# ucsdarclab/Python-SuPer

Measured on AMD Instinct MI355X. Metric: LM iterations/s (embedded-deformation LM, point-to-plane + ARAP + Rot), higher is better.
Workload: dtype f64

## Files before the change

python-super_amd/csrc/slm_api.hip:

```cpp
#include <atomic>
#include <condition_variable>
#include <functional>
#include <mutex>
#include <new>
#include <string>
#include <thread>
#include <algorithm>
#include <vector>
#include <cstdio>
#include <cstring>

#include "slm_common.h"
#include "slm_corr.h"
#include "slm_host.h"
#include "slm_launch.h"
#include "slm_prep.h"

static thread_local std::string g_err;
static const char* const kBadKnn =
    "slm_bind_frame: a KNN index (sf_knn_idx or ed_knn_idx) lies outside [0, J) or a surfel's row of sf_knn_idx repeats an id";

void slm_set_error_text(const char* msg) { g_err = msg; }

namespace {
// ... 195 lines not shown
  void ensure(int n_workers) {
    while ((int)threads_.size() < n_workers) {
      const int id = (int)threads_.size();
      threads_.emplace_back([this, id] { loop(id); });
    }
  }
  void loop(int id) {
    int seen = 0;
    for (;;) {
      const std::function<void(int)>* job = nullptr;
      {
        std::unique_lock<std::mutex> lk(m_);
        cv_work_.wait(lk, [&] { return stop_ || generation_ != seen; });
        if (stop_) return;
        seen = generation_;
        if (id < n_active_) job = job_;
      }
      if (job) {
        (*job)(id + 1);
        std::lock_guard<std::mutex> lk(m_);
        if (--pending_ == 0) cv_done_.notify_all();
      }
    }
  }
  std::vector<std::thread> threads_;
  std::mutex m_;
  std::condition_variable cv_work_, cv_done_;
  const std::function<void(int)>* job_ = nullptr;
  int generation_ = 0, n_active_ = 0, pending_ = 0;
  bool stop_ = false;
};
}

struct slm_solver {
  PrepBuffers* prep = nullptr;
  BindPool bind_pool;
  AsyncWorker prep_worker;
  PrepBuffers* prep_async = nullptr;
  hipStream_t prep_stream = nullptr;
  std::vector<PrepBuffers*> bind_prep;
  std::vector<hipStream_t> bind_streams;
  std::vector<hipEvent_t> bind_events;
  std::mutex band_mutex;
  hipEvent_t drain_event = nullptr;
  double drain_est_ms = 0.0;
  int last_solver_form = -1;
  int last_dag_mode = -1;
  bool no_reuse = false;
  bool hybrid_batches = true;
  long dag_max_nodes = 8000;
  bool fuse_begin = true;
  int gram_wgs = 0;
  int n_cus = 256;
  bool pure_fill = true;
  bool profile = false;
  std::vector<hipEvent_t> ev_pool;
  std::vector<std::vector<hipEvent_t>> ev_runs;
  slm_config cfg{};
  std::vector<Slot> slots;
  FrameDev* frames_dev = nullptr;
  int* bw_dev = nullptr;
  int* bw_host = nullptr;
  int* reuse_dev = nullptr;
  int rank = 0, world = 1;
  int corr_mode = 0;
  double corr_w = 0.0;
  CorrDev* corr_dev = nullptr;
  bool shard_mode = false;
};
namespace {
bool solve_is_task_graph(const slm_solver* s, int n, int J);
}

static std::atomic<long long> g_reallocs{0}, g_realloc_bytes{0}, g_plan_builds{0}, g_plan_reuses{0}, g_plan_fill_hits{0};

template <typename T>
static hipError_t grow(T*& p, size_t& cap, size_t need) {
  if (need <= cap) return hipSuccess;
  const size_t want = need + need / 8;
  ++g_reallocs;
  g_realloc_bytes += (long long)(want * sizeof(T));
  return grow(p, cap, need, want);
}
template <typename T>
static hipError_t grow(GP<T>& p, size_t& cap, size_t need) {
  T* q = p;
  const hipError_t e = grow(q, cap, need);
  p = q;
  return e;
}

static int check_slots(slm_solver* s, int first, int n);

extern "C" {

const char* slm_last_error(void) { return g_err.c_str(); }

int slm_debug_last_solver_form(slm_solver* s) { return s ? s->last_solver_form : -1; }
int slm_debug_last_dag_mode(slm_solver* s) { return s ? s->last_dag_mode : -1; }

int slm_debug_counters(int64_t out[4]) {
  if (!out) return fail(SLM_ERR_INVALID, "slm_debug_counters: null output");
  out[0] = g_reallocs;
  out[1] = g_realloc_bytes;
  out[2] = g_plan_builds;
  out[3] = g_plan_reuses;
// ... 107 lines not shown
    return fail(SLM_ERR_INVALID, buf);
  }
  return SLM_OK;
}

int slm_device_count(void) {
  int n = 0;
  if (hipGetDeviceCount(&n) != hipSuccess) return 0;
  return n;
}

int slm_create(const slm_config* cfg, slm_solver** out) {
  if (!cfg || !out) return fail(SLM_ERR_INVALID, "slm_create: null argument");
  if (cfg->max_frames < 1 || cfg->num_iterations < 0 || !(cfg->v > 0.0))
    return fail(SLM_ERR_INVALID, "slm_create: bad config");
  if (cfg->solver_path < 0 || cfg->solver_path > 4) return fail(SLM_ERR_INVALID, "slm_create: solver_path must be 0..4");
  if (cfg->data_path < 0 || cfg->data_path > 2) return fail(SLM_ERR_INVALID, "slm_create: data_path must be 0..2");
  if (slm_device_count() < 1) return fail(SLM_ERR_NO_DEVICE, "slm_create: no HIP device visible");
  slm_solver* s = new (std::nothrow) slm_solver();
  if (!s) return fail(SLM_ERR_HIP, "slm_create: out of host memory");
  s->cfg = *cfg;
  try {
    s->slots.resize(cfg->max_frames);
  } catch (...) {
    delete s;
    return fail(SLM_ERR_HIP, "slm_create: out of host memory");
  }
  hipError_t e = hipMalloc((void**)&s->frames_dev, sizeof(FrameDev) * cfg->max_frames);
  if (e == hipSuccess) e = hipMemset(s->frames_dev, 0, sizeof(FrameDev) * cfg->max_frames);
  if (e == hipSuccess) e = hipMalloc((void**)&s->bw_dev, 2 * sizeof(int));
  if (e == hipSuccess) e = hipMalloc((void**)&s->reuse_dev, sizeof(int) * cfg->max_frames);
  if (e == hipSuccess) e = hipMemset(s->reuse_dev, 0, sizeof(int) * cfg->max_frames);
  if (e == hipSuccess) e = hipHostMalloc((void**)&s->bw_host, 2 * sizeof(int), hipHostMallocDefault);
  if (e == hipSuccess) {
    s->prep = prep_create();
    if (!s->prep) e = hipErrorOutOfMemory;
  }
  if (e != hipSuccess) {
    g_err = std::string("slm_create: ") + hipGetErrorString(e);
    slm_destroy(s);
    return SLM_ERR_HIP;
  }
  {
    int dev = 0;
    (void)hipGetDevice(&dev);
    (void)dag_device_setup(dev, nullptr);
  }
  if (const char* hb = getenv("SLM_HYBRID")) s->hybrid_batches = atoi(hb) != 0;
  if (const char* dm = getenv("SLM_DAG_MAX_NODES")) s->dag_max_nodes = atol(dm);
  if (const char* nr = getenv("SLM_NO_REUSE")) s->no_reuse = atoi(nr) != 0;
  if (const char* pf = getenv("SLM_PURE_FILL")) s->pure_fill = atoi(pf) != 0;
  if (const char* fb = getenv("SLM_FUSE_BEGIN")) s->fuse_begin = atoi(fb) != 0;
  if (const char* gw = getenv("SLM_GRAM_WGS")) s->gram_wgs = std::min(std::max(atoi(gw), 0), 65535);
  {
    int dev = 0, cus = 0;
    (void)hipGetDevice(&dev);
    if (hipDeviceGetAttribute(&cus, hipDeviceAttributeMultiprocessorCount, dev) == hipSuccess && cus > 0) s->n_cus = cus;
  }
  *out = s;
  return SLM_OK;
}

int slm_destroy(slm_solver* s) {
  if (!s) return SLM_OK;
  s->prep_worker.shutdown();
  s->bind_pool.shutdown();
  for (Slot& sl : s->slots) {
    FrameDev& h = sl.h;
    if (h.beta) (void)hipFree(h.beta);
    if (h.delta) (void)hipFree(h.delta);
    if (h.rhs) (void)hipFree(h.rhs);
    if (sl.band) (void)hipFree(sl.band);
    if (sl.linv) (void)hipFree(sl.linv);
    if (h.loss_part) (void)hipFree(h.loss_part);
    if (h.st) (void)hipFree(h.st);
    if (h.rec) (void)hipFree(h.rec);
    if (h.node_pk) (void)hipFree(h.node_pk);
    if (h.tgt_pn) (void)hipFree(h.tgt_pn);
    if (h.tgt_px) (void)hipFree(h.tgt_px);
    if (h.ev_rc) (void)hipFree(h.ev_rc);
    plan_free(sl.plan);
    pairplan_free(sl.pplan);
    if (sl.h_pin) (void)hipHostFree(sl.h_pin);
    sl.h_pairs.release();
    sl.h_knn.release();
    sl.h_pts.release();
    sl.h_pts64.release();
    if (sl.d_fronts) (void)hipFree(sl.d_fronts);
    if (sl.d_items) (void)hipFree(sl.d_items);
    if (sl.d_tile_kind) (void)hipFree(sl.d_tile_kind);
    if (sl.d_zero_tiles) (void)hipFree(sl.d_zero_tiles);
    if (sl.d_ints) (void)hipFree(sl.d_ints);
    if (sl.d_dests) (void)hipFree(sl.d_dests);
    if (sl.d_cur_dests) (void)hipFree(sl.d_cur_dests);
    if (sl.ftiles) (void)hipFree(sl.ftiles);
    if (sl.fvec) (void)hipFree(sl.fvec);
    if (sl.flinv) (void)hipFree(sl.flinv);
    if (sl.fmail) (void)hipFree(sl.fmail);
    if (sl.pairbuf) (void)hipFree(sl.pairbuf);
    if (sl.corr.o) (void)hipFree(sl.corr.o);
    if (sl.corr.n) (void)hipFree(sl.corr.n);
    if (sl.corr.valid) (void)hipFree(sl.corr.valid);
    if (sl.d_dag_flags) (void)hipFree(sl.d_dag_flags);
    if (sl.d_dag_trace) (void)hipFree(sl.d_dag_trace);
    if (sl.prep_fork) (void)hipEventDestroy(sl.prep_fork);
    if (sl.prep_done) (void)hipEventDestroy(sl.prep_done);
// ... 704 lines not shown
  d.fused_begin = d.nd && tuple && d.gram_variants == 1 && d.max_pos > 0 && s->fuse_begin;
  if (tuple && c.phase_test) d.accept_reuse = s->reuse_dev + first;
  d.accept_eval = tuple ? 1 : 0;
  if (d.nd) {
    for (int i = first; i < first + n; ++i) {
      const auto& sc = s->slots[i].cache.nd.sched;
      if (sc.size() > d.sched.size()) d.sched.resize(sc.size(), NDLevelSched{0, 0, 0, 0, 0, -2, 0, -2, 0, -2});
      for (size_t l = 0; l < sc.size(); ++l) {
        NDLevelSched& m = d.sched[l];
        if (m.first == -2) m.first = sc[l].first;
        else if (m.first != sc[l].first || m.n_fronts != sc[l].n_fronts) m.first = -1;
        m.n_fronts = std::max(m.n_fronts, sc[l].n_fronts);
        m.max_npt = std::max(m.max_npt, sc[l].max_npt);
        m.max_nt = std::max(m.max_nt, sc[l].max_nt);
        m.max_pairs = std::max(m.max_pairs, sc[l].max_pairs);
        m.max_n2p = std::max(m.max_n2p, sc[l].max_n2p);
        if (m.schur_at == -2) m.schur_at = sc[l].schur_at;
        else if (m.schur_at != sc[l].schur_at || m.n_schur != sc[l].n_schur) m.schur_at = -1;
        m.n_schur = std::max(m.n_schur, sc[l].n_schur);
        if (m.pull_at == -2) m.pull_at = sc[l].pull_at;
        else if (m.pull_at != sc[l].pull_at || m.n_pull != sc[l].n_pull) m.pull_at = -1;
        m.n_pull = std::max(m.n_pull, sc[l].n_pull);
      }
    }
  }
  if (d.nd && n > 1) {
    for (int i = first; i < first + n; ++i)
      for (size_t l = s->slots[i].cache.nd.sched.size(); l < d.sched.size(); ++l)
        d.sched[l].first = d.sched[l].schur_at = d.sched[l].pull_at = -1;
  }
  for (auto& m : d.sched) {
    if (m.first == -2) m.first = -1;
    if (m.first < 0) m.schur_at = m.pull_at = -1;
    if (m.schur_at == -2) m.schur_at = -1;
    if (m.pull_at == -2) m.pull_at = -1;
  }
  if (s->cfg.use_arap || s->cfg.use_rot)
    d.n_reg_part = std::min(kRegBlocksMax, (d.maxJKe + 255) / 256);
  d.n_acc_part = d.n_reg_part + (s->corr_mode ? kCorrBlocks : 0);
  return d;
}

static bool solve_is_task_graph(const slm_solver* s, int n, int J) {
  return s->cfg.solver_path == 2 || (s->cfg.solver_path == 0 && (n <= 2 || (long)n * J <= s->dag_max_nodes));
}
static bool solve_is_hybrid(const slm_solver* s, int n, const BatchDims& d) {
  return !solve_is_task_graph(s, n, d.maxP / 7) && (s->cfg.solver_path == 4 || (s->cfg.solver_path == 0 && s->hybrid_batches)) &&
         d.hybrid_cut >= 0 && d.hybrid_levels == (int)d.sched.size() && d.hybrid_cut + 1 < d.hybrid_levels;
}
static int dag_cut_of(const slm_solver* s, int n, const BatchDims& d) {
  if (solve_is_task_graph(s, n, d.maxP / 7)) return -1;
  return solve_is_hybrid(s, n, d) ? d.hybrid_cut : -2;
}
int enqueue_front_solve(slm_solver* s, const FrameDev* fr, int n, const BatchDims& d, double u_override, hipStream_t st,
                        bool dag_reset_done = false, bool dag_check_later = false) {
  const bool dag = solve_is_task_graph(s, n, d.maxP / 7);
  const bool hybrid = solve_is_hybrid(s, n, d);
  s->last_solver_form = dag ? 1 : (hybrid ? 2 : 0);
  int mode = -1;
  if (dag) {
    mode = launch_front_solve_dag(fr, n, d.max_tasks, u_override, st, -1, !dag_reset_done, !dag_check_later);
  } else if (hybrid) {
    const int n_levels = (int)d.sched.size(), l_cut = n_levels - 1 - d.hybrid_cut;
    launch_front_levels(fr, n, d.sched.data(), n_levels, l_cut, 0, u_override, st);
    mode = launch_front_solve_dag(fr, n, d.max_top_tasks, u_override, st, d.hybrid_cut, !dag_reset_done, !dag_check_later);
  } else {
    launch_front_solve(fr, n, d.sched.data(), (int)d.sched.size(), u_override, st);
  }
  s->last_dag_mode = mode;
  return mode;
}

void enqueue_zero(const FrameDev* fr, int n, const BatchDims& d, hipStream_t st, const int* reuse, int dag_cut, bool fused) {
  if (!d.nd) launch_iter_begin(fr, n, st);
  else if (!fused) launch_iter_begin_nd(fr, n, st, reuse, dag_cut);
}

void enqueue_jacobian(slm_solver* s, const FrameDev* fr, int n, const BatchDims& d, hipStream_t st, int eval_mode,
                      const int* reuse, int dag_cut, bool fused) {
  const double w = s->cfg.w_data;
  switch (d.form) {
    case DataForm::tuple:
      if (eval_mode >= 0) launch_data_eval(fr, n, kLossBlocks, w, eval_mode, st, reuse);
      if (fused) launch_begin_and_gram(fr, n, w, st, reuse, dag_cut, s->gram_wgs, s->n_cus);
      else launch_data_gram(fr, n, d.max_pos, w, d.gram_variants, st, reuse, s->gram_wgs, s->n_cus);
      break;
    case DataForm::pairs:
      launch_data_grad_pairs(fr, n, d.maxN, d.K, w, st);
      if (d.corr) launch_corr_grad_pairs(fr, s->corr_dev + (fr - s->frames_dev), n, d.maxN, d.K, s->corr_mode, s->corr_w, st);
      break;
    case DataForm::per_entry:
      launch_data_grad(fr, n, d.maxN, d.K, w, st);
      if (d.corr) launch_corr_grad(fr, s->corr_dev + (fr - s->frames_dev), n, d.maxN, d.K, s->corr_mode, s->corr_w, st);
      break;
    case DataForm::none: break;
  }
}

enum class Shard { whole, before_exchange, after_exchange };
void enqueue_scatter(slm_solver* s, const FrameDev* fr, int n, const BatchDims& d, hipStream_t st, Shard part) {
  const slm_config& c = s->cfg;
  const bool tuple = d.form == DataForm::tuple;
  if (part == Shard::before_exchange) {
    if (tuple) launch_pair_reduce(fr, n, d.max_blocks, st);
    return;
  }
  if (part == Shard::after_exchange || d.form == DataForm::pairs) launch_pair_scatter(fr, n, d.max_blocks, st);
  else if (tuple && d.nd) launch_front_assemble(fr, n, d.max_blocks, st);
  else if (tuple) launch_band_assemble(fr, n, d.max_blocks, st);
  if (d.nd) {
    launch_reg_grad_nd(fr, n, d.maxP / 7, c.use_arap, c.w_arap, c.use_rot, c.w_rot, st);
    if (!c.use_arap && !c.use_rot) launch_front_load_rhs(fr, n, d.maxP, st);
  } else {
    launch_reg_grad(fr, n, d.maxJKe, c.use_arap, c.w_arap, c.use_rot, c.w_rot, st);
  }
}

void enqueue_data_loss(slm_solver* s, const FrameDev* fr, int n, const BatchDims& d, hipStream_t st, bool at_beta) {
  if (d.form == DataForm::tuple && !at_beta) launch_data_eval(fr, n, kLossBlocks, s->cfg.w_data, 0, st);
  else if (d.form != DataForm::none) launch_data_loss(fr, n, kLossBlocks, d.K, s->cfg.w_data, at_beta ? 0 : 1, st);
// ... 630 lines not shown
```

python-super_amd/csrc/slm_front.hip:

```cpp
#include <algorithm>
#include <atomic>
#include <cstdlib>

#include "slm_tile.h"
#include "slm_begin.h"
#include "slm_launch.h"

__device__ __forceinline__ int nd_base(const NDFront& f, int p) {
  return p < f.nv ? 7 * p : f.n1p + 7 * (p - f.nv);
}

__device__ __forceinline__ double* ftile(const FrameDev& fd, const NDFront& f, int r, int c) {
  const size_t t = (size_t)c * f.nt - (size_t)c * (c - 1) / 2 + (size_t)(r - c);
  return fd.ftiles + f.tile_off + t * TILE;
}

__device__ __forceinline__ double* front_entry(const FrameDev& fd, const NDFront& f, int i, int j) {
  return ftile(fd, f, i >> 6, j >> 6) + (i & 63) + (size_t)(j & 63) * NB;
}

__device__ __forceinline__ double* dest_entry(const FrameDev& fd, const NDDest& d, int x, int y) {
  const NDFront& f = fd.fronts[d.front];
  const int rb = nd_base(f, d.prow), cb = nd_base(f, d.pcol);
  return d.transpose ? front_entry(fd, f, rb + y, cb + x) : front_entry(fd, f, rb + x, cb + y);
// ... 385 lines not shown
                                                 int c, double u_override, WgMap map) {
  extern __shared__ double lds[];
  double *S = PanelLds::S(lds), *M = PanelLds::M(lds), *dinv = PanelLds::dinv(lds), *vec = PanelLds::vec(lds);
  LevelCtx cx;
  if (!level_begin(frames, lvl, c, map, cx)) return;
  const FrameDev& fd = *cx.fd;
  const NDFront& f = *cx.f;
  const int d = cx.unit;
  if (c + d >= f.nt) return;
  const double u = (u_override >= 0.0) ? u_override : fd.st->u;
  const bool stamp = (c == 1 && cx.frame == 0 && cx.front == 0 && d == 1 && lvl.level == fd.n_levels - 1);
  SLM_STAMP(fd, stamp, 0);
  double* At = ftile(fd, f, c + d, c);
  double* yv = fd.fvec + f.vec_off + (size_t)c * NB;
  double4_t a[4];
  panel_column_stage(d, At, yv, ftile(fd, f, c, c), c * NB, f.n1, u, S, vec, a);
  SLM_STAMP(fd, stamp, 1);
  const bool ok = PanelLds::factor(lds, nullptr, nullptr, nullptr, min(4, (f.n1 - c * NB + 15) >> 4));
  SLM_STAMP(fd, stamp, 14);
  if (d == 0 && !ok && threadIdx.x == 0) fd.st->chol_fail = 1;
  panel_column_finish(d, At, yv, fd.flinv + f.linv_off + (size_t)c * TILE, S, M, dinv, vec, a);
  SLM_STAMP(fd, stamp, 15);
}

__global__ void __launch_bounds__(256) k_fpotrf(const FrameDev* __restrict__ frames, LevelRef lvl, int c,
                                                 double u_override) {
  extern __shared__ double lds[];
  double *S = PanelLds::S(lds), *M = PanelLds::M(lds), *dinv = PanelLds::dinv(lds), *vec = PanelLds::vec(lds);
  LevelCtx cx;
  if (!level_begin(frames, lvl, c, cx)) return;
  const FrameDev& fd = *cx.fd;
  const NDFront& f = *cx.f;
  const double u = (u_override >= 0.0) ? u_override : fd.st->u;
  double* yv = fd.fvec + f.vec_off + (size_t)c * NB;
  double4_t a[4];
  panel_column_stage(0, nullptr, yv, ftile(fd, f, c, c), c * NB, f.n1, u, S, vec, a);
  const bool ok = PanelLds::factor(lds, nullptr, nullptr, nullptr, min(4, (f.n1 - c * NB + 15) >> 4));
  if (!ok && threadIdx.x == 0) fd.st->chol_fail = 1;
  panel_column_finish(0, nullptr, yv, fd.flinv + f.linv_off + (size_t)c * TILE, S, M, dinv, vec, a);
}

__global__ void __launch_bounds__(256) k_ftrsm(const FrameDev* __restrict__ frames, LevelRef lvl, int c, WgMap map) {
  __shared__ double Bl[TILE];
  LevelCtx cx;
  if (!level_begin(frames, lvl, c, map, cx)) return;
  const FrameDev& fd = *cx.fd;
  const NDFront& f = *cx.f;
  const int d = cx.unit + 1;
  if (c + d >= f.nt) return;
  double* At = ftile(fd, f, c + d, c);
  tile_product<false, true, false>(fd.flinv + f.linv_off + (size_t)c * TILE, At, At, Bl);
}

__device__ __forceinline__ const NDTileItem* tile_item(const FrameDev* __restrict__ frames, int level, int which, int n_items,
                                                       int at, int n_frames, const FrameDev*& fdp) {
  const int total = n_items * n_frames;
  const int chunk = (total + 7) >> 3;
  const int q = blockIdx.x >> 3;
  const int w_id = (blockIdx.x & 7) * chunk + q;
  if (q >= chunk || w_id >= total) return nullptr;
  const int frame = w_id / n_items, item_idx = w_id - frame * n_items;
  const FrameDev& fd = frames[frame];
  if (!fd.bound || !fd.nd_ready) return nullptr;
  int i0 = at;
  if (at < 0) {
    if (level >= fd.n_levels) return nullptr;
    i0 = fd.item_off[2 * level + which];
    if (item_idx >= fd.item_off[2 * level + which + 1] - i0) return nullptr;
  }
  fdp = &fd;
  return fd.tile_items.get() + i0 + item_idx;
}
__device__ __forceinline__ NDTileItem item_snapshot(const NDTileItem* p) {
  NDTileItem o;
  const int* src = reinterpret_cast<const int*>(p);
  int* dst = reinterpret_cast<int*>(&o);
#pragma unroll
  for (int i = 0; i < (int)(sizeof(NDTileItem) / 4); ++i) dst[i] = __builtin_amdgcn_readfirstlane(src[i]);
  return o;
}
__device__ __forceinline__ double* item_tile(const FrameDev& fd, const NDTileItem& it, int r, int c) {
  const size_t t = (size_t)c * it.nt - (size_t)c * (c - 1) / 2 + (size_t)(r - c);
  return fd.ftiles + (c < it.npt ? it.tile_off : it.f22_base) + t * TILE;
}
__device__ __forceinline__ void pull_maps(const FrameDev& fd, const NDTileItem& it, int2* maps) {
#pragma unroll
  for (int k = 0; k < 2; ++k) {
    if (it.kid[k].front >= 0 && threadIdx.x < 128) {
      const int32_t* pm = fd.pullmap + it.kid[k].pull_off;
      const bool row = threadIdx.x < 64;
      const int c = pm[64 * (row ? it.r : it.c) + (threadIdx.x & 63)];
      int off = 0;
      if (c >= 0) {
        const int t = it.kid[k].npt + (c >> 6);
        off = row ? t * TILE + (c & 63) : (t * it.kid[k].nt - t * (t - 1) / 2 - t) * TILE + (c & 63) * NB;
      }
      maps[128 * k + threadIdx.x] = make_int2(c, off);
    }
  }
}
__device__ __forceinline__ void pull_tile(const FrameDev& fd, const NDTileItem& it, const int2* maps, double4_t acc[4]) {
  const int l = threadIdx.x & 63, w = threadIdx.x >> 6, lr = l & 15, lk = l >> 4;
#pragma unroll
  for (int k = 0; k < 2; ++k) {
    if (it.kid[k].front < 0) continue;
    __builtin_amdgcn_sched_barrier(0);
    double v[16];
    const double* ct = fd.ftiles + it.kid[k].f22_base;
    const int2* mk = maps + 128 * k;
    const int2 rw = mk[16 * w + lr];
#pragma unroll
    for (int ni = 0; ni < 4; ++ni)
#pragma unroll
      for (int rr = 0; rr < 4; ++rr) {
        const int2 cl = mk[64 + 16 * ni + lk + 4 * rr];
        const bool ok = cl.x >= 0 && rw.x >= cl.x;
        const double x = ct[ok ? rw.y + cl.y : 0];
        v[4 * ni + rr] = ok ? x : 0.0;
      }
    __builtin_amdgcn_sched_barrier(0);
#pragma unroll
    for (int ni = 0; ni < 4; ++ni)
#pragma unroll
      for (int rr = 0; rr < 4; ++rr) acc[ni][rr] += v[4 * ni + rr];
    __builtin_amdgcn_sched_barrier(0);
  }
}
__device__ __forceinline__ double pull_vec(const FrameDev& fd, const NDTileItem& it, const int2* maps) {
  double s = 0.0;
  if (threadIdx.x < NB) {
#pragma unroll
    for (int k = 0; k < 2; ++k) {
      if (it.kid[k].front < 0) continue;
      const int ci = maps[128 * k + threadIdx.x].x;
      if (ci >= 0) s += fd.fvec[it.kid[k].vec_boundary + ci];
    }
  }
  return s;
}

__global__ void __launch_bounds__(256, 2) k_fL11(const FrameDev* __restrict__ frames, LevelRef lvl,
                                               double u_override) {
  extern __shared__ double lds[];
  double *S = L11Lds::S(lds), *M = L11Lds::M(lds);
  double* Bl = L11Lds::Bl(lds);
  double* vec = L11Lds::vec(lds);
  double* part = L11Lds::vec2(lds);
  LevelCtx cx;
  if (!level_begin(frames, lvl, 0, cx)) return;
  const FrameDev& fd = *cx.fd;
  const NDFront& f = *cx.f;
  const double u = (u_override >= 0.0) ? u_override : fd.st->u;
  double* vecs = fd.fvec + f.vec_off;
  const int w = threadIdx.x >> 6, l = threadIdx.x & 63, lr = l & 15, lk = l >> 4;

  for (int c = 0; c < f.npt; ++c) {
    double rhs_c = 0.0;
    {
      double v[16];
      tile_to_regs(ftile(fd, f, c, c), v);
      if (threadIdx.x < NB) rhs_c = vecs[(size_t)c * NB + threadIdx.x];
#pragma unroll
      for (int t = 0; t < 16; ++t) {
        const int e = threadIdx.x + 256 * t;
        const int i = e % NB, k = e / NB;
        double x = (i >= k) ? v[t] : 0.0;
        if (i == k) x = (c * NB + i < f.n1) ? x + u : 1.0;
        S[i + k * LD] = x;
      }
    }
    __syncthreads();
    const bool ok = L11Lds::factor(lds, nullptr, nullptr, nullptr, min(4, (f.n1 - c * NB + 15) >> 4));
    if (!ok && threadIdx.x == 0) fd.st->chol_fail = 1;
    if (threadIdx.x < NB) vec[threadIdx.x] = rhs_c;
    __syncthreads();
    {
      commit_pivot(M, vec, fd.flinv + f.linv_off + (size_t)c * TILE, part);
      __syncthreads();
      if (threadIdx.x < NB) {
        vec[threadIdx.x] = part[threadIdx.x];
        vecs[(size_t)c * NB + threadIdx.x] = part[threadIdx.x];
      }
      __syncthreads();
    }
    for (int r = c + 1; r < f.npt; ++r) {
      double* At = ftile(fd, f, r, c);
      double areg[16];
// ... 91 lines not shown
  LevelCtx cx;
  if (!level_begin(frames, lvl, c, map, cx)) return;
  const FrameDev& fd = *cx.fd;
  const NDFront& f = *cx.f;
  const int m = f.nt - 1 - c;
  int t = cx.unit;
  if (t < ntile_cap) {
    int db = 1;
    while (db <= bcap && t >= mcap - db + 1) {
      t -= mcap - db + 1;
      ++db;
    }
    const int da = db + t;
    if (da > m || c + db >= f.npt) return;
    tile_product<true, false, true>(ftile(fd, f, c + db, c), ftile(fd, f, c + da, c), ftile(fd, f, c + da, c + db), Bl);
  } else {
    const int db = t - ntile_cap + 1;
    if (db > m) return;
    __shared__ double y[NB];
    __shared__ double part[4 * NB];
    double* vecs = fd.fvec + f.vec_off;
    trail_rhs(ftile(fd, f, c + db, c), vecs + (size_t)c * NB, vecs + (size_t)(c + db) * NB, y, part);
  }
}

__global__ void __launch_bounds__(256) k_fpull(const FrameDev* __restrict__ frames, int level, int n_items, int items_at,
                                                int n_frames) {
  __shared__ int2 maps[256];
  const FrameDev* fdp;
  const NDTileItem* itp = tile_item(frames, level, 1, n_items, items_at, n_frames, fdp);
  if (!itp) return;
  const FrameDev& fd = *fdp;
  const NDTileItem it = item_snapshot(itp);
  const int w = threadIdx.x >> 6;
  const int vrow = it.r < it.npt ? min(NB, it.n1 - NB * it.r) : min(NB, it.n2 - NB * (it.r - it.npt));
  const int nblk = (min(NB, it.n1 - NB * it.c) + 15) >> 4;
  const bool wave_on = 16 * w < vrow;
  pull_maps(fd, it, maps);
  double* T = item_tile(fd, it, it.r, it.c);
  const bool pure = __builtin_amdgcn_readfirstlane((int)fd.tile_kind[it.pad0]) != 0;
  double4_t acc[4];
  zero_acc(acc);
  if (wave_on && !pure) load_c_frags_nblk(T, acc, nblk);
  __syncthreads();
  if (wave_on) pull_tile(fd, it, maps, acc);
  if (pure) store_c_frags(T, acc);
  else if (wave_on) store_c_frags_nblk(T, acc, nblk);
  if (it.r == it.c) {
    const double v = pull_vec(fd, it, maps);
    if (threadIdx.x < NB && v != 0.0) fd.fvec[it.vec_off + (size_t)it.c * NB + threadIdx.x] += v;
  }
}

__global__ void __launch_bounds__(256, 3) k_fschur(const FrameDev* __restrict__ frames, int level, int n_items,
                                                 int items_at, int n_frames) {
  __shared__ __attribute__((aligned(16))) double Bl[TILE];
  __shared__ int2 maps[256];
  const FrameDev* fdp;
  const NDTileItem* itp = tile_item(frames, level, 0, n_items, items_at, n_frames, fdp);
  if (!itp) return;
  const FrameDev& fd = *fdp;
  const NDTileItem& it = *itp;
  const int r = it.r, sc = it.c, tr = r - it.npt, tc = sc - it.npt;
  const int l = threadIdx.x & 63, w = threadIdx.x >> 6, lr = l & 15, lk = l >> 4;
  const int vrow = min(NB, it.n2 - NB * tr), vcol = min(NB, it.n2 - NB * tc);
  const bool wave_on = 16 * w < vrow;
  const int nblk = (tr == tc) ? min((vcol + 15) >> 4, w + 1) : (vcol + 15) >> 4;
  const bool kids = it.kid[0].front >= 0 || it.kid[1].front >= 0;
  pull_maps(fd, it, maps);
  typedef double dvec2 __attribute__((ext_vector_type(2)));
  dvec2 breg[4];
  double areg[16], acur[16];
  if (it.npt > 0) {
    const dvec2* Ls = reinterpret_cast<const dvec2*>(item_tile(fd, it, sc, 0));
#pragma unroll
    for (int e = 0; e < 4; ++e) breg[e] = Ls[threadIdx.x + 256 * e];
    if (wave_on) load_a_frags(item_tile(fd, it, r, 0), areg);
  }
  double4_t acc[4];
  zero_acc(acc);
  __syncthreads();
  if (kids) pull_tile(fd, it, maps, acc);
  for (int c = 0; c < it.npt; ++c) {
    const dvec2* Ls = reinterpret_cast<const dvec2*>(item_tile(fd, it, sc, c));
    dvec2* Bl2 = reinterpret_cast<dvec2*>(Bl);
    const int ksteps = min(16, (it.n1 - NB * c + 3) >> 2);
#pragma unroll
    for (int e = 0; e < 4; ++e) Bl2[threadIdx.x + 256 * e] = breg[e];
#pragma unroll
    for (int e = 0; e < 16; ++e) acur[e] = areg[e];
    if (ksteps > 8) {
#pragma unroll
      for (int e = 0; e < 4; ++e) breg[e] = Ls[TILE / 4 + threadIdx.x + 256 * e];
    }
    if (c + 1 < it.npt && wave_on) load_a_frags(item_tile(fd, it, r, c + 1), areg);
    __syncthreads();
    if (wave_on) {
#pragma unroll
      for (int ks = 0; ks < 8; ++ks) {
        if (ks < ksteps) {
          const double av = -acur[ks];
#pragma unroll
          for (int ni = 0; ni < 4; ++ni)
            if (ni < nblk)
              acc[ni] = __builtin_amdgcn_mfma_f64_16x16x4f64(Bl[(16 * ni + lr) + (4 * ks + lk) * LD], av, acc[ni], 0, 0, 0);
        }
      }
    }
    if (ksteps > 8) {
#pragma unroll
      for (int e = 0; e < 4; ++e) Bl2[TILE / 4 + threadIdx.x + 256 * e] = breg[e];
    }
    if (c + 1 < it.npt) {
      const dvec2* Ln = reinterpret_cast<const dvec2*>(item_tile(fd, it, sc, c + 1));
#pragma unroll
      for (int e = 0; e < 4; ++e) breg[e] = Ln[threadIdx.x + 256 * e];
    }
    __syncthreads();
    if (wave_on) {
#pragma unroll
      for (int ks = 8; ks < 16; ++ks) {
        if (ks < ksteps) {
          const double av = -acur[ks];
#pragma unroll
          for (int ni = 0; ni < 4; ++ni)
            if (ni < nblk)
              acc[ni] = __builtin_amdgcn_mfma_f64_16x16x4f64(Bl[(16 * ni + lr) + (4 * ks + lk) * LD], av, acc[ni], 0, 0, 0);
        }
      }
    }
  }
  if (wave_on) store_c_frags_nblk(item_tile(fd, it, r, sc), acc, nblk);
  if (tr == tc && kids) {
    const double v = pull_vec(fd, it, maps);
    if (threadIdx.x < NB && v != 0.0) fd.fvec[it.vec_off + (size_t)r * NB + threadIdx.x] += v;
  }
}

__global__ void __launch_bounds__(256) k_fback_prep(const FrameDev* __restrict__ frames, LevelRef lvl) {
  extern __shared__ double xb[];
  LevelCtx cx;
  if (!level_begin(frames, lvl, blockIdx.x, cx)) return;
  const FrameDev& fd = *cx.fd;
  const NDFront& f = *cx.f;
  const int c = cx.unit;
  if (f.nb == 0) return;
  const int* nodes = fd.nd_nodes + f.nodes_off + f.nv;
  for (int i = threadIdx.x; i < f.n2p; i += blockDim.x)
    xb[i] = (i < 7 * f.nb) ? fd.delta[7 * nodes[i / 7] + i % 7] : 0.0;
  __syncthreads();
  double acc = 0.0;
  for (int r = f.npt; r < f.nt; ++r) acc = tile_t_vec_lanes(ftile(fd, f, r, c), xb + (size_t)(r - f.npt) * NB, acc);
  acc = sum_col_lanes(acc);
  if ((threadIdx.x & 3) == 0) fd.fvec[f.vec_off + (size_t)c * NB + (threadIdx.x >> 2)] -= acc;
}

__global__ void __launch_bounds__(256) k_fbacksub(const FrameDev* __restrict__ frames, LevelRef lvl,
                                                   int step) {
  LevelCtx cx;
  if (!level_begin(frames, lvl, step, cx)) return;
  const FrameDev& fd = *cx.fd;
  const NDFront& f = *cx.f;
  const int c = f.npt - 1 - step;
  const int d = cx.unit;
  if (d > c) return;
  __shared__ double y[NB];
  __shared__ double x[NB];
  __shared__ double part[4 * NB];
  double* vecs = fd.fvec + f.vec_off;
  backsub_x(fd.flinv + f.linv_off + (size_t)c * TILE, vecs + (size_t)c * NB, y, x, part);
  if (d == 0) {
    if (threadIdx.x < NB) {
      const int i = c * NB + threadIdx.x;
      if (i < f.n1) {
        const int node = fd.nd_nodes[f.nodes_off + i / 7];
        fd.delta[7 * node + i % 7] = x[threadIdx.x];
      }
    }
  } else {
    backsub_update(ftile(fd, f, c, c - d), x, vecs + (size_t)(c - d) * NB);
  }
}

void launch_pair_reduce(const FrameDev* fr, int n_frames, int max_blocks, hipStream_t st) {
  if (max_blocks <= 0) return;
  hipLaunchKernelGGL(k_pair_reduce, dim3((max_blocks + 3) / 4, n_frames), dim3(256), 0, st, fr);
}

void launch_pair_scatter(const FrameDev* fr, int n_frames, int max_blocks, hipStream_t st) {
  if (max_blocks <= 0) return;
  hipLaunchKernelGGL(k_pair_scatter, dim3((max_blocks + 3) / 4, n_frames), dim3(256), 0, st, fr);
}

void launch_front_assemble(const FrameDev* fr, int n_frames, int max_blocks, hipStream_t st) {
  if (max_blocks <= 0) return;
  hipLaunchKernelGGL(k_front_assemble, dim3((max_blocks + 3) / 4, n_frames), dim3(256), 0, st, fr);
}

void launch_reg_grad_nd(const FrameDev* fr, int n_frames, int maxJ, int use_arap, double lam_a,
                        int use_rot, double lam_r, hipStream_t st) {
  if (maxJ <= 0 || (!use_arap && !use_rot)) return;
  hipLaunchKernelGGL(k_reg_grad_nd, dim3((maxJ * RG_LANES + 255) / 256, n_frames), dim3(256), 0, st, fr, use_arap,
                     lam_a, use_rot, lam_r);
}

void launch_front_load_rhs(const FrameDev* fr, int n_frames, int maxP, hipStream_t st) {
  hipLaunchKernelGGL(k_front_load_rhs, dim3((maxP + 255) / 256, n_frames), dim3(256), 0, st, fr);
}

void launch_iter_begin_nd(const FrameDev* fr, int n_frames, hipStream_t st, const int* reuse, int dag_cut) {
  hipLaunchKernelGGL(k_iter_begin_nd, dim3(1024, n_frames), dim3(256), 0, st, fr, reuse, dag_cut);
}

bool ensure_dynamic_lds(const void* kernel, size_t bytes) {
  static std::atomic<const void*> done[64][8];
  int dev = 0;
  (void)hipGetDevice(&dev);
  const bool tracked = dev >= 0 && dev < 64;
  if (tracked)
    for (auto& slot : done[dev])
      if (slot.load(std::memory_order_acquire) == kernel) return true;
  if (hipFuncSetAttribute(kernel, hipFuncAttributeMaxDynamicSharedMemorySize, (int)bytes) != hipSuccess) return false;
  if (tracked)
    for (auto& slot : done[dev]) {
      const void* seen = nullptr;
      if (slot.compare_exchange_strong(seen, kernel, std::memory_order_acq_rel) || seen == kernel) break;
    }
  return true;
}

void launch_front_levels(const FrameDev* fr, int n_frames, const NDLevelSched* lv, int n_levels, int l_factor_end,
                         int l_back_end, double u_override, hipStream_t st) {
  const size_t lds = PANEL_LDS_DOUBLES * sizeof(double);
  const size_t lds11 = L11_LDS_DOUBLES * sizeof(double);
  if (!ensure_dynamic_lds((const void*)k_fL11, lds11) || !ensure_dynamic_lds((const void*)k_fpanel, lds) ||
      !ensure_dynamic_lds((const void*)k_fpotrf, lds))
    return;
  static const long compact_min = [] {
    const char* e = getenv("SLM_COMPACT_MIN");
    return e ? atol(e) : 64L;
  }();
  static const int compact_npt = [] {
    const char* e = getenv("SLM_COMPACT_NPT");
    return e ? atoi(e) : 4;
  }();
  for (int l = 0; l < l_factor_end; ++l) {
    const NDLevelSched& s = lv[l];
    if (s.n_fronts <= 0) continue;
    const LevelRef lr{l, s.first, s.n_fronts};
    const bool compact = s.max_npt <= compact_npt && (long)s.n_fronts * n_frames >= compact_min;
    if (s.n_pull > 0) {
      const int total = s.n_pull * n_frames;
      hipLaunchKernelGGL(k_fpull, dim3((unsigned)((total + 7) / 8 * 8)), dim3(256), 0, st, fr, l, s.n_pull, s.pull_at, n_frames);
    }
    if (compact) {
      hipLaunchKernelGGL(k_fL11, dim3(1, s.n_fronts, n_frames), dim3(256), lds11, st, fr, lr, u_override);
      if (s.max_n2p > 0) {
        const WgMap m = make_map(s.max_n2p / 64, s.n_fronts, n_frames);
        hipLaunchKernelGGL(k_fL21, map_grid(m), dim3(256), 0, st, fr, lr, m);
      }
    }
    for (int c = 0; !compact && c < s.max_npt; ++c) {
      const int mcap = s.max_nt - 1 - c;
      if ((long)(mcap + 1) * s.n_fronts * n_frames <= 512) {
        const WgMap m = make_map(mcap + 1, s.n_fronts, n_frames);
        hipLaunchKernelGGL(k_fpanel, map_grid(m), dim3(256), lds, st, fr, lr, c, u_override, m);
      } else {
        hipLaunchKernelGGL(k_fpotrf, dim3(1, s.n_fronts, n_frames), dim3(256), lds, st, fr, lr, c,
                           u_override);
        if (mcap > 0) {
          const WgMap m = make_map(mcap, s.n_fronts, n_frames);
          hipLaunchKernelGGL(k_ftrsm, map_grid(m), dim3(256), 0, st, fr, lr, c, m);
        }
      }
      const int bcap = std::min(mcap, s.max_npt - 1 - c);
      int ntile = 0;
      for (int b = 1; b <= bcap; ++b) ntile += mcap - b + 1;
      if (ntile + mcap > 0) {
        const WgMap m = make_map(ntile + mcap, s.n_fronts, n_frames);
        hipLaunchKernelGGL(k_ftrail, map_grid(m), dim3(256), 0, st, fr, lr, c, mcap, bcap, ntile, m);
      }
    }
    if (s.n_schur > 0) {
      const int total = s.n_schur * n_frames;
      hipLaunchKernelGGL(k_fschur, dim3((unsigned)((total + 7) / 8 * 8)), dim3(256), 0, st, fr, l, s.n_schur, s.schur_at,
                         n_frames);
    }
  }
  for (int l = l_back_end - 1; l >= 0; --l) {
    const NDLevelSched& s = lv[l];
    if (s.n_fronts <= 0 || s.max_npt <= 0) continue;
    const LevelRef lr{l, s.first, s.n_fronts};
    if (s.max_n2p > 0)
      hipLaunchKernelGGL(k_fback_prep, dim3(s.max_npt, s.n_fronts, n_frames), dim3(256),
                         (size_t)s.max_n2p * sizeof(double), st, fr, lr);
    for (int e = 0; e < s.max_npt; ++e)
      hipLaunchKernelGGL(k_fbacksub, dim3(s.max_npt, s.n_fronts, n_frames), dim3(256), 0, st, fr,
                         lr, e);
  }
}

void launch_front_solve(const FrameDev* fr, int n_frames, const NDLevelSched* lv, int n_levels,
                        double u_override, hipStream_t st) {
  launch_front_levels(fr, n_frames, lv, n_levels, n_levels, 0, u_override, st);
  launch_front_levels(fr, n_frames, lv, n_levels, 0, n_levels, u_override, st);
}
```

python-super_amd/csrc/slm_launch.h:

```cpp
#pragma once
#include "slm_common.h"

void launch_data_grad(const FrameDev*, int, int, int, double, hipStream_t);
void launch_data_grad_pairs(const FrameDev*, int, int, int, double, hipStream_t);
void launch_data_loss(const FrameDev*, int, int, int, double, int, hipStream_t);
void launch_data_resid(const FrameDev*, int, int, int, double, double*, uint8_t*, int32_t*, hipStream_t);

void launch_data_gram(const FrameDev*, int, int, double, int, hipStream_t, const int* reuse, int wgs, int n_cus);
void launch_begin_and_gram(const FrameDev*, int, double, hipStream_t, const int* reuse, int dag_cut, int wgs, int n_cus);
void launch_data_eval(const FrameDev*, int, int, double, int mode, hipStream_t, const int* reuse = nullptr);
void launch_band_assemble(const FrameDev*, int, int, hipStream_t);

void launch_front_assemble(const FrameDev*, int, int, hipStream_t);
void launch_pair_reduce(const FrameDev*, int, int, hipStream_t);
void launch_pair_scatter(const FrameDev*, int, int, hipStream_t);
void launch_reg_grad_nd(const FrameDev*, int, int, int, double, int, double, hipStream_t);
void launch_front_load_rhs(const FrameDev*, int, int, hipStream_t);
void launch_iter_begin_nd(const FrameDev*, int, hipStream_t, const int* reuse, int dag_cut);
void launch_front_solve(const FrameDev*, int, const NDLevelSched*, int, double, hipStream_t);
void launch_front_levels(const FrameDev*, int, const NDLevelSched*, int, int, int, double, hipStream_t);

bool ensure_dynamic_lds(const void* kernel, size_t bytes);

int launch_front_solve_dag(const FrameDev*, int, int, double, hipStream_t, int cut, bool reset, bool check);
int dag_device_setup(int dev, int* xcd8_out);
int dag_last_mode();
hipError_t set_dag_timeout_ticks(long long);
void launch_dag_abort_check(const FrameDev*, int, hipStream_t);

void launch_bandwidth(const slm_frame&, int*, hipStream_t);
void launch_band_solve(const FrameDev*, int, int, int, double, hipStream_t);
void launch_band_to_dense(const FrameDev*, int, double*, hipStream_t);
void launch_dense_to_band(const FrameDev*, const double*, const double*, hipStream_t);

void launch_reg_grad(const FrameDev*, int, int, int, double, int, double, hipStream_t);
void launch_after_solve(const FrameDev*, int, int, int, int, double, int, double, int, hipStream_t);
void launch_reg_loss(const FrameDev*, int, int, int, double, int, double, int, hipStream_t);

void launch_init_slot(const FrameDev*, int, int, const slm_config&, hipStream_t);
void launch_iter_begin(const FrameDev*, int, hipStream_t);
void launch_pack_nodes(const FrameDev*, int, int, hipStream_t);
void launch_make_trial(const FrameDev*, int, int, hipStream_t);
void launch_pack_target(int, const float*, const float*, float4*, hipStream_t);
void launch_pack_target_px(int, const int*, const uint8_t*, const float*, const float*, float4*, hipStream_t);
void launch_accept(const FrameDev*, int, int, int, int, hipStream_t, int* reuse = nullptr, int eval_pass = 0);
void launch_loss_out(const FrameDev*, int, int, double*, hipStream_t);
void launch_zero_reg_part(const FrameDev*, int, int, hipStream_t);
void launch_update(int, int, int, float*, float*, const int*, const float*, float*, float*, const double*, hipStream_t);
void launch_update64(int, int, int, double*, double*, const int*, const double*, double*, double*, const double*,
                     hipStream_t);
void launch_knn(int, int, int, int, const float*, const float*, int*, float*, hipStream_t);
void launch_knn64(int, int, int, int, const double*, const double*, const int*, const int*, int*, double*, int*,
                  hipStream_t);
void launch_knn_weights64(int, int, int, const int*, const double*, const double*, int, const double*, const double*,
                          double*, uint8_t*, hipStream_t);
void launch_knn_weights(int, int, int, const int*, const float*, const float*, float*, uint8_t*, hipStream_t);
```

Baseline: 3398.

## Make Schur update kernel persistent with cross-item prefetch of tiles and maps

The front Schur-complement kernel becomes a persistent grid of at most 4×CU workgroups that walks over several tile items. While it finishes one item it prefetches the next item's pull maps and first A/B tiles into registers and a double-buffered LDS map, and it loads item and frame metadata through scalar loads. Occupancy is raised from 3 to 4 waves per SIMD. The aim is to cut launch tail, per-item setup latency and the number of workgroups, at the cost of more register pressure and a more complex control flow.

```diff
diff --git a/python-super_amd/csrc/slm_api.hip b/python-super_amd/csrc/slm_api.hip
--- a/python-super_amd/csrc/slm_api.hip
+++ b/python-super_amd/csrc/slm_api.hip
@@ -271,6 +271,7 @@
   bool fuse_begin = true;
   int gram_wgs = 0;
   int n_cus = 256;
+  int schur_wgs = -1;
   bool pure_fill = true;
   bool profile = false;
   std::vector<hipEvent_t> ev_pool;
@@ -484,6 +485,7 @@
   if (const char* pf = getenv("SLM_PURE_FILL")) s->pure_fill = atoi(pf) != 0;
   if (const char* fb = getenv("SLM_FUSE_BEGIN")) s->fuse_begin = atoi(fb) != 0;
   if (const char* gw = getenv("SLM_GRAM_WGS")) s->gram_wgs = std::min(std::max(atoi(gw), 0), 65535);
+  if (const char* sw = getenv("SLM_SCHUR_WGS")) s->schur_wgs = std::min(std::max(atoi(sw), 0), 1 << 20);
   {
     int dev = 0, cus = 0;
     (void)hipGetDevice(&dev);
@@ -1294,6 +1296,7 @@
   if (solve_is_task_graph(s, n, d.maxP / 7)) return -1;
   return solve_is_hybrid(s, n, d) ? d.hybrid_cut : -2;
 }
+static int schur_wgs_of(const slm_solver* s) { return s->schur_wgs >= 0 ? s->schur_wgs : 4 * s->n_cus; }
 int enqueue_front_solve(slm_solver* s, const FrameDev* fr, int n, const BatchDims& d, double u_override, hipStream_t st,
                         bool dag_reset_done = false, bool dag_check_later = false) {
   const bool dag = solve_is_task_graph(s, n, d.maxP / 7);
@@ -1304,10 +1307,10 @@
     mode = launch_front_solve_dag(fr, n, d.max_tasks, u_override, st, -1, !dag_reset_done, !dag_check_later);
   } else if (hybrid) {
     const int n_levels = (int)d.sched.size(), l_cut = n_levels - 1 - d.hybrid_cut;
-    launch_front_levels(fr, n, d.sched.data(), n_levels, l_cut, 0, u_override, st);
+    launch_front_levels(fr, n, d.sched.data(), n_levels, l_cut, 0, u_override, st, schur_wgs_of(s));
     mode = launch_front_solve_dag(fr, n, d.max_top_tasks, u_override, st, d.hybrid_cut, !dag_reset_done, !dag_check_later);
   } else {
-    launch_front_solve(fr, n, d.sched.data(), (int)d.sched.size(), u_override, st);
+    launch_front_solve(fr, n, d.sched.data(), (int)d.sched.size(), u_override, st, schur_wgs_of(s));
   }
   s->last_dag_mode = mode;
   return mode;
diff --git a/python-super_amd/csrc/slm_front.hip b/python-super_amd/csrc/slm_front.hip
--- a/python-super_amd/csrc/slm_front.hip
+++ b/python-super_amd/csrc/slm_front.hip
@@ -461,11 +461,10 @@
   tile_product<false, true, false>(fd.flinv + f.linv_off + (size_t)c * TILE, At, At, Bl);
 }
 
-__device__ __forceinline__ const NDTileItem* tile_item(const FrameDev* __restrict__ frames, int level, int which, int n_items,
-                                                       int at, int n_frames, const FrameDev*& fdp) {
+__device__ __forceinline__ const NDTileItem* tile_item_at(const FrameDev* __restrict__ frames, int level, int which, int n_items,
+                                                          int at, int n_frames, int q, const FrameDev*& fdp) {
   const int total = n_items * n_frames;
   const int chunk = (total + 7) >> 3;
-  const int q = blockIdx.x >> 3;
   const int w_id = (blockIdx.x & 7) * chunk + q;
   if (q >= chunk || w_id >= total) return nullptr;
   const int frame = w_id / n_items, item_idx = w_id - frame * n_items;
@@ -480,6 +479,17 @@
   fdp = &fd;
   return fd.tile_items.get() + i0 + item_idx;
 }
+__device__ __forceinline__ const NDTileItem* tile_item(const FrameDev* __restrict__ frames, int level, int which, int n_items,
+                                                       int at, int n_frames, const FrameDev*& fdp) {
+  return tile_item_at(frames, level, which, n_items, at, n_frames, blockIdx.x >> 3, fdp);
+}
+__device__ __forceinline__ const NDTileItem* tile_item_walk(const FrameDev* __restrict__ frames, int level, int which, int n_items,
+                                                            int at, int n_frames, int& q, const FrameDev*& fdp) {
+  const int chunk = (n_items * n_frames + 7) >> 3, nq = gridDim.x >> 3;
+  for (q += nq; q < chunk; q += nq)
+    if (const NDTileItem* p = tile_item_at(frames, level, which, n_items, at, n_frames, q, fdp)) return p;
+  return nullptr;
+}
 __device__ __forceinline__ NDTileItem item_snapshot(const NDTileItem* p) {
   NDTileItem o;
   const int* src = reinterpret_cast<const int*>(p);
@@ -488,28 +498,55 @@
   for (int i = 0; i < (int)(sizeof(NDTileItem) / 4); ++i) dst[i] = __builtin_amdgcn_readfirstlane(src[i]);
   return o;
 }
-__device__ __forceinline__ double* item_tile(const FrameDev& fd, const NDTileItem& it, int r, int c) {
+template <class T>
+__device__ __forceinline__ T load_scalars(const T* p) {
+  static_assert(sizeof(T) % 4 == 0, "whole words");
+  typedef const __attribute__((address_space(4))) int* kptr;
+  const kptr src = (kptr) reinterpret_cast<const int*>(p);
+  T o;
+  int* dst = reinterpret_cast<int*>(&o);
+#pragma unroll
+  for (int i = 0; i < (int)(sizeof(T) / 4); ++i) dst[i] = src[i];
+  return o;
+}
+template <class FD>
+__device__ __forceinline__ double* item_tile(const FD& fd, const NDTileItem& it, int r, int c) {
   const size_t t = (size_t)c * it.nt - (size_t)c * (c - 1) / 2 + (size_t)(r - c);
   return fd.ftiles + (c < it.npt ? it.tile_off : it.f22_base) + t * TILE;
 }
-__device__ __forceinline__ void pull_maps(const FrameDev& fd, const NDTileItem& it, int2* maps) {
+template <class FD>
+__device__ __forceinline__ void pull_maps_load(const FD& fd, const NDTileItem& it, int c[2], int tid = threadIdx.x) {
 #pragma unroll
   for (int k = 0; k < 2; ++k) {
-    if (it.kid[k].front >= 0 && threadIdx.x < 128) {
-      const int32_t* pm = fd.pullmap + it.kid[k].pull_off;
-      const bool row = threadIdx.x < 64;
-      const int c = pm[64 * (row ? it.r : it.c) + (threadIdx.x & 63)];
+    c[k] = -1;
+    if (it.kid[k].front >= 0 && tid < 128)
+      c[k] = fd.pullmap[it.kid[k].pull_off + 64 * (tid < 64 ? it.r : it.c) + (tid & 63)];
+  }
+}
+__device__ __forceinline__ void pull_maps_store(const NDTileItem& it, const int cs[2], int2* maps, int tid = threadIdx.x) {
+#pragma unroll
+  for (int k = 0; k < 2; ++k) {
+    if (it.kid[k].front >= 0 && tid < 128) {
+      const bool row = tid < 64;
+      const int c = cs[k];
       int off = 0;
       if (c >= 0) {
         const int t = it.kid[k].npt + (c >> 6);
         off = row ? t * TILE + (c & 63) : (t * it.kid[k].nt - t * (t - 1) / 2 - t) * TILE + (c & 63) * NB;
       }
-      maps[128 * k + threadIdx.x] = make_int2(c, off);
-    }
-  }
-}
-__device__ __forceinline__ void pull_tile(const FrameDev& fd, const NDTileItem& it, const int2* maps, double4_t acc[4]) {
-  const int l = threadIdx.x & 63, w = threadIdx.x >> 6, lr = l & 15, lk = l >> 4;
+      maps[128 * k + tid] = make_int2(c, off);
+    }
+  }
+}
+template <class FD>
+__device__ __forceinline__ void pull_maps(const FD& fd, const NDTileItem& it, int2* maps) {
+  int c[2];
+  pull_maps_load(fd, it, c);
+  pull_maps_store(it, c, maps);
+}
+template <class FD>
+__device__ __forceinline__ void pull_tile(const FD& fd, const NDTileItem& it, const int2* maps, double4_t acc[4], int tid = threadIdx.x) {
+  const int l = tid & 63, w = tid >> 6, lr = l & 15, lk = l >> 4;
 #pragma unroll
   for (int k = 0; k < 2; ++k) {
     if (it.kid[k].front < 0) continue;
@@ -535,13 +572,14 @@
     __builtin_amdgcn_sched_barrier(0);
   }
 }
-__device__ __forceinline__ double pull_vec(const FrameDev& fd, const NDTileItem& it, const int2* maps) {
+template <class FD>
+__device__ __forceinline__ double pull_vec(const FD& fd, const NDTileItem& it, const int2* maps, int tid = threadIdx.x) {
   double s = 0.0;
-  if (threadIdx.x < NB) {
+  if (tid < NB) {
 #pragma unroll
     for (int k = 0; k < 2; ++k) {
       if (it.kid[k].front < 0) continue;
-      const int ci = maps[128 * k + threadIdx.x].x;
+      const int ci = maps[128 * k + tid].x;
       if (ci >= 0) s += fd.fvec[it.kid[k].vec_boundary + ci];
     }
   }
@@ -739,88 +777,161 @@
   }
 }
 
-__global__ void __launch_bounds__(256, 3) k_fschur(const FrameDev* __restrict__ frames, int level, int n_items,
+typedef double dvec2 __attribute__((ext_vector_type(2)));
+struct SchurBase {
+  GP<double> ftiles, fvec;
+  GP<const int32_t> pullmap;
+};
+__device__ __forceinline__ SchurBase schur_base(const FrameDev* fd) {
+  SchurBase b;
+  b.ftiles = load_scalars(&fd->ftiles);
+  b.fvec = load_scalars(&fd->fvec);
+  b.pullmap = load_scalars(&fd->pullmap);
+  return b;
+}
+__device__ __forceinline__ int lane_tid() {
+  int t = threadIdx.x;
+  asm volatile("" : "+v"(t));
+  return t;
+}
+__device__ __forceinline__ void schur_load_a(const double* __restrict__ A, int tid, double areg[16]) {
+  const int l = tid & 63, w = tid >> 6, lr = l & 15, lk = l >> 4;
+#pragma unroll
+  for (int ks = 0; ks < 16; ++ks) areg[ks] = A[(unsigned)((16 * w + lr) + (4 * ks + lk) * NB)];
+}
+__device__ __forceinline__ void schur_load_b(const double* __restrict__ L, int tid, dvec2 breg[4]) {
+  const dvec2* L2 = reinterpret_cast<const dvec2*>(L);
+#pragma unroll
+  for (int e = 0; e < 4; ++e) breg[e] = L2[(unsigned)(tid + 256 * e)];
+}
+__device__ __forceinline__ void schur_store_c(double* Cg, int tid, const double4_t acc[4], int nblk) {
+  const int l = tid & 63, w = tid >> 6, lr = l & 15, lk = l >> 4;
+#pragma unroll
+  for (int ni = 0; ni < 4; ++ni)
+    if (ni < nblk) {
+#pragma unroll
+      for (int rr = 0; rr < 4; ++rr) Cg[(unsigned)((16 * w + lr) + (16 * ni + lk + 4 * rr) * NB)] = acc[ni][rr];
+    }
+}
+__device__ __forceinline__ void schur_first_b(const SchurBase& fd, const NDTileItem& it, int tid, dvec2 breg[4]) {
+  if (it.npt > 0) schur_load_b(item_tile(fd, it, it.c, 0), tid, breg);
+}
+__device__ __forceinline__ void schur_first_a(const SchurBase& fd, const NDTileItem& it, int tid, int w, double areg[16]) {
+  if (it.npt > 0 && 16 * w < min(NB, it.n2 - NB * (it.r - it.npt))) schur_load_a(item_tile(fd, it, it.r, 0), tid, areg);
+}
+__global__ void __launch_bounds__(256, 4) k_fschur(const FrameDev* __restrict__ frames, int level, int n_items,
                                                  int items_at, int n_frames) {
   __shared__ __attribute__((aligned(16))) double Bl[TILE];
-  __shared__ int2 maps[256];
-  const FrameDev* fdp;
-  const NDTileItem* itp = tile_item(frames, level, 0, n_items, items_at, n_frames, fdp);
+  __shared__ int2 maps2[2][256];
+  const FrameDev* fdp = nullptr;
+  int q = (int)(blockIdx.x >> 3) - (int)(gridDim.x >> 3);
+  const NDTileItem* itp = tile_item_walk(frames, level, 0, n_items, items_at, n_frames, q, fdp);
   if (!itp) return;
-  const FrameDev& fd = *fdp;
-  const NDTileItem& it = *itp;
-  const int r = it.r, sc = it.c, tr = r - it.npt, tc = sc - it.npt;
-  const int l = threadIdx.x & 63, w = threadIdx.x >> 6, lr = l & 15, lk = l >> 4;
-  const int vrow = min(NB, it.n2 - NB * tr), vcol = min(NB, it.n2 - NB * tc);
-  const bool wave_on = 16 * w < vrow;
-  const int nblk = (tr == tc) ? min((vcol + 15) >> 4, w + 1) : (vcol + 15) >> 4;
-  const bool kids = it.kid[0].front >= 0 || it.kid[1].front >= 0;
-  pull_maps(fd, it, maps);
-  typedef double dvec2 __attribute__((ext_vector_type(2)));
+  const int w = __builtin_amdgcn_readfirstlane(threadIdx.x >> 6);
   dvec2 breg[4];
   double areg[16], acur[16];
-  if (it.npt > 0) {
-    const dvec2* Ls = reinterpret_cast<const dvec2*>(item_tile(fd, it, sc, 0));
-#pragma unroll
-    for (int e = 0; e < 4; ++e) breg[e] = Ls[threadIdx.x + 256 * e];
-    if (wave_on) load_a_frags(item_tile(fd, it, r, 0), areg);
-  }
-  double4_t acc[4];
-  zero_acc(acc);
-  __syncthreads();
-  if (kids) pull_tile(fd, it, maps, acc);
-  for (int c = 0; c < it.npt; ++c) {
-    const dvec2* Ls = reinterpret_cast<const dvec2*>(item_tile(fd, it, sc, c));
-    dvec2* Bl2 = reinterpret_cast<dvec2*>(Bl);
-    const int ksteps = min(16, (it.n1 - NB * c + 3) >> 2);
-#pragma unroll
-    for (int e = 0; e < 4; ++e) Bl2[threadIdx.x + 256 * e] = breg[e];
-#pragma unroll
-    for (int e = 0; e < 16; ++e) acur[e] = areg[e];
-    if (ksteps > 8) {
-#pragma unroll
-      for (int e = 0; e < 4; ++e) breg[e] = Ls[TILE / 4 + threadIdx.x + 256 * e];
-    }
-    if (c + 1 < it.npt && wave_on) load_a_frags(item_tile(fd, it, r, c + 1), areg);
+  {
+    const NDTileItem it = load_scalars(itp);
+    const SchurBase fd = schur_base(fdp);
+    int m0[2];
+    pull_maps_load(fd, it, m0, lane_tid());
+    pull_maps_store(it, m0, maps2[0], lane_tid());
+    schur_first_b(fd, it, lane_tid(), breg);
+    schur_first_a(fd, it, lane_tid(), w, areg);
+  }
+  for (int buf = 0;; buf ^= 1) {
+    const int2* maps = maps2[buf];
+    const NDTileItem it = load_scalars(itp);
+    const SchurBase fd = schur_base(fdp);
+    const int r = it.r, sc = it.c, tr = r - it.npt, tc = sc - it.npt;
+    const int vrow = min(NB, it.n2 - NB * tr), vcol = min(NB, it.n2 - NB * tc);
+    const bool wave_on = 16 * w < vrow;
+    const int nblk = (tr == tc) ? min((vcol + 15) >> 4, w + 1) : (vcol + 15) >> 4;
+    const bool kids = it.kid[0].front >= 0 || it.kid[1].front >= 0;
+    double4_t acc[4];
+    zero_acc(acc);
     __syncthreads();
-    if (wave_on) {
-#pragma unroll
-      for (int ks = 0; ks < 8; ++ks) {
-        if (ks < ksteps) {
-          const double av = -acur[ks];
-#pragma unroll
-          for (int ni = 0; ni < 4; ++ni)
-            if (ni < nblk)
-              acc[ni] = __builtin_amdgcn_mfma_f64_16x16x4f64(Bl[(16 * ni + lr) + (4 * ks + lk) * LD], av, acc[ni], 0, 0, 0);
+    if (kids) pull_tile(fd, it, maps, acc, lane_tid());
+    __builtin_amdgcn_sched_barrier(0);
+    itp = tile_item_walk(frames, level, 0, n_items, items_at, n_frames, q, fdp);
+    const bool more = itp != nullptr;
+    NDTileItem nit = it;
+    SchurBase nfd = fd;
+    if (more) {
+      nit = load_scalars(itp);
+      nfd = schur_base(fdp);
+    }
+    __builtin_amdgcn_sched_barrier(0);
+    int nmap[2] = {-1, -1};
+    if (it.npt <= 0 && more) {
+      pull_maps_load(nfd, nit, nmap, lane_tid());
+      schur_first_b(nfd, nit, lane_tid(), breg);
+      schur_first_a(nfd, nit, lane_tid(), w, areg);
+    }
+    for (int c = 0; c < it.npt; ++c) {
+      const bool last = c + 1 >= it.npt;
+      const int tid = lane_tid(), lr = tid & 15, lk = (tid >> 4) & 3;
+      const dvec2* Ls = reinterpret_cast<const dvec2*>(item_tile(fd, it, sc, c));
+      dvec2* Bl2 = reinterpret_cast<dvec2*>(Bl);
+      const int ksteps = min(16, (it.n1 - NB * c + 3) >> 2);
+#pragma unroll
+      for (int e = 0; e < 4; ++e) Bl2[tid + 256 * e] = breg[e];
+#pragma unroll
+      for (int e = 0; e < 16; ++e) acur[e] = areg[e];
+      if (ksteps > 8) {
+#pragma unroll
+        for (int e = 0; e < 4; ++e) breg[e] = Ls[(unsigned)(TILE / 4 + tid + 256 * e)];
+      }
+      if (!last) {
+        if (wave_on) schur_load_a(item_tile(fd, it, r, c + 1), tid, areg);
+      } else if (more) {
+        pull_maps_load(nfd, nit, nmap, tid);
+        schur_first_a(nfd, nit, tid, w, areg);
+      }
+      __syncthreads();
+      if (wave_on) {
+#pragma unroll
+        for (int ks = 0; ks < 8; ++ks) {
+          if (ks < ksteps) {
+            const double av = -acur[ks];
+#pragma unroll
+            for (int ni = 0; ni < 4; ++ni)
+              if (ni < nblk)
+                acc[ni] = __builtin_amdgcn_mfma_f64_16x16x4f64(Bl[(16 * ni + lr) + (4 * ks + lk) * LD], av, acc[ni], 0, 0, 0);
+          }
         }
       }
-    }
-    if (ksteps > 8) {
-#pragma unroll
-      for (int e = 0; e < 4; ++e) Bl2[TILE / 4 + threadIdx.x + 256 * e] = breg[e];
-    }
-    if (c + 1 < it.npt) {
-      const dvec2* Ln = reinterpret_cast<const dvec2*>(item_tile(fd, it, sc, c + 1));
-#pragma unroll
-      for (int e = 0; e < 4; ++e) breg[e] = Ln[threadIdx.x + 256 * e];
-    }
-    __syncthreads();
-    if (wave_on) {
-#pragma unroll
-      for (int ks = 8; ks < 16; ++ks) {
-        if (ks < ksteps) {
-          const double av = -acur[ks];
-#pragma unroll
-          for (int ni = 0; ni < 4; ++ni)
-            if (ni < nblk)
-              acc[ni] = __builtin_amdgcn_mfma_f64_16x16x4f64(Bl[(16 * ni + lr) + (4 * ks + lk) * LD], av, acc[ni], 0, 0, 0);
+      if (ksteps > 8) {
+#pragma unroll
+        for (int e = 0; e < 4; ++e) Bl2[TILE / 4 + tid + 256 * e] = breg[e];
+      }
+      if (!last) {
+        schur_load_b(item_tile(fd, it, sc, c + 1), tid, breg);
+      } else if (more) {
+        schur_first_b(nfd, nit, tid, breg);
+      }
+      __syncthreads();
+      if (wave_on) {
+#pragma unroll
+        for (int ks = 8; ks < 16; ++ks) {
+          if (ks < ksteps) {
+            const double av = -acur[ks];
+#pragma unroll
+            for (int ni = 0; ni < 4; ++ni)
+              if (ni < nblk)
+                acc[ni] = __builtin_amdgcn_mfma_f64_16x16x4f64(Bl[(16 * ni + lr) + (4 * ks + lk) * LD], av, acc[ni], 0, 0, 0);
+          }
         }
       }
     }
-  }
-  if (wave_on) store_c_frags_nblk(item_tile(fd, it, r, sc), acc, nblk);
-  if (tr == tc && kids) {
-    const double v = pull_vec(fd, it, maps);
-    if (threadIdx.x < NB && v != 0.0) fd.fvec[it.vec_off + (size_t)r * NB + threadIdx.x] += v;
+    if (more) pull_maps_store(nit, nmap, maps2[buf ^ 1], lane_tid());
+    if (wave_on) schur_store_c(item_tile(fd, it, r, sc), lane_tid(), acc, nblk);
+    if (tr == tc && kids) {
+      const int tid = lane_tid();
+      const double v = pull_vec(fd, it, maps, tid);
+      if (tid < NB && v != 0.0) fd.fvec[it.vec_off + (size_t)r * NB + tid] += v;
+    }
+    if (!more) break;
   }
 }
 
@@ -917,7 +1028,7 @@
 }
 
 void launch_front_levels(const FrameDev* fr, int n_frames, const NDLevelSched* lv, int n_levels, int l_factor_end,
-                         int l_back_end, double u_override, hipStream_t st) {
+                         int l_back_end, double u_override, hipStream_t st, int schur_wgs) {
   const size_t lds = PANEL_LDS_DOUBLES * sizeof(double);
   const size_t lds11 = L11_LDS_DOUBLES * sizeof(double);
   if (!ensure_dynamic_lds((const void*)k_fL11, lds11) || !ensure_dynamic_lds((const void*)k_fpanel, lds) ||
@@ -970,8 +1081,9 @@
     }
     if (s.n_schur > 0) {
       const int total = s.n_schur * n_frames;
-      hipLaunchKernelGGL(k_fschur, dim3((unsigned)((total + 7) / 8 * 8)), dim3(256), 0, st, fr, l, s.n_schur, s.schur_at,
-                         n_frames);
+      int wgs = (total + 7) / 8 * 8;
+      if (schur_wgs > 0) wgs = std::min(wgs, (schur_wgs + 7) / 8 * 8);
+      hipLaunchKernelGGL(k_fschur, dim3((unsigned)wgs), dim3(256), 0, st, fr, l, s.n_schur, s.schur_at, n_frames);
     }
   }
   for (int l = l_back_end - 1; l >= 0; --l) {
@@ -988,7 +1100,7 @@
 }
 
 void launch_front_solve(const FrameDev* fr, int n_frames, const NDLevelSched* lv, int n_levels,
-                        double u_override, hipStream_t st) {
-  launch_front_levels(fr, n_frames, lv, n_levels, n_levels, 0, u_override, st);
-  launch_front_levels(fr, n_frames, lv, n_levels, 0, n_levels, u_override, st);
-}
+                        double u_override, hipStream_t st, int schur_wgs) {
+  launch_front_levels(fr, n_frames, lv, n_levels, n_levels, 0, u_override, st, schur_wgs);
+  launch_front_levels(fr, n_frames, lv, n_levels, 0, n_levels, u_override, st, schur_wgs);
+}
diff --git a/python-super_amd/csrc/slm_launch.h b/python-super_amd/csrc/slm_launch.h
--- a/python-super_amd/csrc/slm_launch.h
+++ b/python-super_amd/csrc/slm_launch.h
@@ -17,8 +17,8 @@
 void launch_reg_grad_nd(const FrameDev*, int, int, int, double, int, double, hipStream_t);
 void launch_front_load_rhs(const FrameDev*, int, int, hipStream_t);
 void launch_iter_begin_nd(const FrameDev*, int, hipStream_t, const int* reuse, int dag_cut);
-void launch_front_solve(const FrameDev*, int, const NDLevelSched*, int, double, hipStream_t);
-void launch_front_levels(const FrameDev*, int, const NDLevelSched*, int, int, int, double, hipStream_t);
+void launch_front_solve(const FrameDev*, int, const NDLevelSched*, int, double, hipStream_t, int schur_wgs);
+void launch_front_levels(const FrameDev*, int, const NDLevelSched*, int, int, int, double, hipStream_t, int schur_wgs);
 
 bool ensure_dynamic_lds(const void* kernel, size_t bytes);
 
```

Result: slower. 3356 (-1.2%).
